# ChristophReich1996/Semantic_Pyramid_for_Image_Generation

Hardware: AMD Instinct MI355X
Metric: images/sec full G+D train step, 256x256, bs/GPU=20 (higher is better)
Workload: dtype bf16

## Files before the change

include/sempyr.h:

```cpp
#ifndef SEMPYR_H
#define SEMPYR_H
#include <stdint.h>

#ifdef __cplusplus
extern "C" {
#endif

#define SP_VERSION 1

typedef void* sp_stream_t;

enum sp_status { SP_OK = 0, SP_ERR_INVALID = -1, SP_ERR_LAUNCH = -2, SP_ERR_UNSUPPORTED = -3 };
enum sp_dtype { SP_F32 = 0, SP_BF16 = 1, SP_F8 = 2 ,
                SP_F16 = 3 ,
                SP_F8_F16 = 4  };
enum sp_act { SP_ACT_NONE = 0, SP_ACT_LRELU = 1, SP_ACT_RELU = 2, SP_ACT_TANH = 3 };

int sp_version(void);

enum { SP_TUNE_CONV_TALL = 0, SP_TUNE_IGEMM_DMA = 1, SP_TUNE_WGRAD_ROWS = 2, SP_TUNE_DETERMINISTIC = 3,
       SP_TUNE_SPLITK_TARGET = 4, SP_TUNE_SPLITK_MINSTEPS = 5, SP_TUNE_CONV1X1_DIRECT = 6, SP_TUNE_CONV_SHORT = 7,
       SP_TUNE_WGRAD9_BLOCKS = 8, SP_TUNE_WGRAD_BLOCKS = 9, SP_TUNE_WGRAD_MINSTEPS = 10, SP_TUNE_WGRAD_SMALL_M = 11,
       SP_TUNE_WGRAD_K1_TILE64 = 12, SP_TUNE_WGRAD_ROWS_THIN = 13, SP_TUNE_WGRAD_ROWS_BLOCKS = 14, SP_TUNE_WGRAD_ROWS_SLABS = 15,
       SP_TUNE_CONV_STAGGER = 16, SP_TUNE_CONV1X1_SPLITK = 17, SP_TUNE_WGRAD1X1 = 18, SP_TUNE_CONV_CIN8 = 19, SP_TUNE_CONV_THINCO = 20, SP_TUNE_CONV_PP = 21, SP_TUNE_CONV_PP_PRIO = 22, SP_TUNE_WGRAD_PP = 23, SP_TUNE_BN_ITERS = 24, SP_TUNE_IGEMM_TILE = 25, SP_TUNE_CONV_PPW = 26, SP_TUNE_LINEAR_KS = 27, SP_TUNE_CONV_PP_SPLIT = 28, SP_TUNE_PAIRSET_SEGMENTS = 29, SP_TUNE_ATTN_PIECES = 30, SP_TUNE_COUNT = 31 };
int sp_set_tuning(int32_t key, int32_t value);
const char* sp_last_error_string(void);
const char* sp_last_route(void);

typedef struct sp_conv_params {
    const void* x;
    const void* w;
    const float* bias;
    void* y;
    const void* res1;
    const void* res2;
    const void* mask_src;
    float mask_neg_slope;
    int32_t n, h, w_, cin_p, cout, ldy, ksize, act, dtype;
    void* workspace;
    int64_t workspace_bytes;
    int32_t pool2;
    int32_t in_up2;
    const float* x_scale;
    const float* w_scale;
    void* y8;
    const float* y8_inv_scale;
    float* y8_amax;
    const float* img_scale;
    int32_t img_split;
    int32_t reserved_;
    int64_t split_pix_;
    const void* tail_w;
    const float* tail_bias;
    void* tail_y;
    int32_t tail_cout, tail_act, tail_ld, reserved2_;
    uint32_t* pool_idx;
    int32_t* split_sync;
} sp_conv_params;
#define SP_CONV_SPLIT_SYNC_BYTES 8192
int sp_conv2d_igemm(const sp_conv_params* p, sp_stream_t stream);
int sp_conv2d_workspace(int32_t n, int32_t h, int32_t w_, int32_t cin_p, int32_t cout, int32_t ksize, int32_t dtype,
                        int64_t* bytes_out);
int sp_conv2d_route(const sp_conv_params* p, const char** route);

int sp_conv2d_wgrad(const void* x, const void* dy, float* dw, int32_t n, int32_t h, int32_t w_,
                    int32_t cin_p, int32_t cout, int32_t ld_dy, int32_t ksize, int32_t dtype,
                    sp_stream_t stream);

int sp_conv2d_wgrad_fused(const void* x, const void* dy, float* dw, float* dbias, const void* w_packed, float* dot,
                          float* workspace, int64_t workspace_floats, int32_t n, int32_t h, int32_t w_, int32_t cin_p,
                          int32_t cout, int32_t ld_dy, int32_t ksize, int32_t dtype, sp_stream_t stream);
int sp_conv2d_wgrad_accum(const void* x, const void* dy, float* dw, float* dbias, float* workspace, int64_t workspace_floats,
                          int32_t n, int32_t h, int32_t w_, int32_t cin_p, int32_t cout, int32_t ld_dy, int32_t ksize,
                          int32_t dtype, sp_stream_t stream);
int sp_conv2d_wgrad_accum_pooled(const void* x, const void* dy, float* dw, float* dbias, float* workspace, int64_t workspace_floats,
                                 int32_t n, int32_t h, int32_t w_, int32_t cin_p, int32_t cout, int32_t ld_dy, int32_t ksize,
                                 int32_t dtype, sp_stream_t stream);
int sp_conv2d_wgrad_workspace(int32_t n, int32_t h, int32_t w_, int32_t cin_p, int32_t cout, int32_t ksize,
                              int32_t dtype, int64_t* floats_out);
int sp_conv2d_wgrad_accum_pair(const void* x, const void* dy, float* dw_a, float* dbias_a, float* dw_b, float* dbias_b, float* workspace,
                               int64_t workspace_floats, int32_t n, int32_t split, int32_t h, int32_t w_, int32_t cin_p, int32_t cout,
                               int32_t ld_dy, int32_t ksize, int32_t dy_pooled, int32_t dtype, sp_stream_t stream);
int sp_conv2d_wgrad_route(int32_t n, int32_t split, int32_t h, int32_t w_, int32_t cin_p, int32_t cout, int32_t ld_dy, int32_t ksize,
                          int32_t dy_pooled, int32_t want_dbias, int64_t workspace_floats, int32_t dtype, const char** route);
int sp_wgrad_reduce_defer(int32_t on);
int sp_wgrad_reduce_flush(int32_t run, sp_stream_t stream);
int sp_wgrad_reduce_pending(void);

int sp_linear_fwd(const void* x, int32_t ldx, const void* w_packed, int32_t kp, const float* bias,
                  const void* res, void* y, int32_t ldy, int32_t batch, int32_t k, int32_t n, int32_t act,
                  int32_t dtype, sp_stream_t stream);
int sp_linear_workspace(int32_t batch, int32_t k, int32_t n, int32_t dtype, int64_t* floats_out);
int sp_linear_fwd_ws(const void* x, int32_t ldx, const void* w_packed, int32_t kp, const float* bias,
                     const void* res, void* y, int32_t ldy, int32_t batch, int32_t k, int32_t n, int32_t act,
                     int32_t dtype, float* scratch, sp_stream_t stream);
int sp_linear_wgrad(const void* x, int32_t ldx, const void* dy, int32_t ld_dy, float* dw, int32_t kp,
                    float* dbias, int32_t batch, int32_t k, int32_t n, int32_t dtype, sp_stream_t stream);

typedef struct sp_sn_layer {
    const float* w;
    float* u;
    float* v;
    int64_t scratch_off;
    int64_t part_off;
    int64_t fwd_off;
    int64_t dgrad_off;
    int32_t rows, cols, cin, taps, cin_p, cout_p, kind, pack_block0;
// ... 284 lines not shown
```

semantic_pyramid_for_image_generation_amd/_lib.py:

```python
from __future__ import annotations

import ctypes
import os
import re
from typing import Dict, List, Tuple

_HERE = os.path.dirname(os.path.abspath(__file__))
HEADER = os.path.join(os.path.dirname(_HERE), "include", "sempyr.h")
LIB_PATH = os.environ.get("SEMPYR_LIB") or os.path.join(_HERE, "libsempyr.so")

SP_F32, SP_BF16, SP_F8, SP_F16, SP_F8_F16 = 0, 1, 2, 3, 4
ACT_NONE, ACT_LRELU, ACT_RELU, ACT_TANH = 0, 1, 2, 3

TUNE_KEYS = {"SP_CONV_TALL": 0, "SP_IGEMM_DMA": 1, "SP_WGRAD_ROWS": 2, "SP_DETERMINISTIC": 3, "SP_SPLITK_TARGET": 4,
             "SP_SPLITK_MINSTEPS": 5, "SP_CONV1X1_DIRECT": 6, "SP_CONV_SHORT": 7, "SP_WGRAD9_BLOCKS": 8, "SP_WGRAD_BLOCKS": 9,
             "SP_WGRAD_MINSTEPS": 10, "SP_WGRAD_SMALL_M": 11, "SP_WGRAD_K1_TILE64": 12, "SP_WGRAD_ROWS_THIN": 13,
             "SP_WGRAD_ROWS_BLOCKS": 14, "SP_WGRAD_ROWS_SLABS": 15, "SP_CONV_STAGGER": 16, "SP_CONV1X1_SPLITK": 17, "SP_WGRAD1X1": 18, "SP_CONV_CIN8": 19, "SP_CONV_THINCO": 20,
             "SP_CONV_PP": 21, "SP_CONV_PP_PRIO": 22, "SP_WGRAD_PP": 23, "SP_BN_ITERS": 24, "SP_IGEMM_TILE": 25, "SP_CONV_PPW": 26, "SP_LINEAR_KS": 27, "SP_CONV_PP_SPLIT": 28, "SP_PAIRSET_SEGMENTS": 29, "SP_ATTN_PIECES": 30}


SP_CONV_SPLIT_SYNC_BYTES = 8192


class SpConvParams(ctypes.Structure):
    _fields_ = [("x", ctypes.c_void_p), ("w", ctypes.c_void_p), ("bias", ctypes.c_void_p), ("y", ctypes.c_void_p),
                ("res1", ctypes.c_void_p), ("res2", ctypes.c_void_p), ("mask_src", ctypes.c_void_p),
                ("mask_neg_slope", ctypes.c_float),
                ("n", ctypes.c_int32), ("h", ctypes.c_int32), ("w_", ctypes.c_int32), ("cin_p", ctypes.c_int32),
                ("cout", ctypes.c_int32), ("ldy", ctypes.c_int32), ("ksize", ctypes.c_int32), ("act", ctypes.c_int32),
                ("dtype", ctypes.c_int32), ("workspace", ctypes.c_void_p), ("workspace_bytes", ctypes.c_int64),
                ("pool2", ctypes.c_int32), ("in_up2", ctypes.c_int32),
                ("x_scale", ctypes.c_void_p), ("w_scale", ctypes.c_void_p), ("y8", ctypes.c_void_p),
                ("y8_inv_scale", ctypes.c_void_p), ("y8_amax", ctypes.c_void_p),
                ("img_scale", ctypes.c_void_p), ("img_split", ctypes.c_int32), ("reserved_", ctypes.c_int32),
                ("split_pix_", ctypes.c_int64),
                ("tail_w", ctypes.c_void_p), ("tail_bias", ctypes.c_void_p), ("tail_y", ctypes.c_void_p),
                ("tail_cout", ctypes.c_int32), ("tail_act", ctypes.c_int32), ("tail_ld", ctypes.c_int32), ("reserved2_", ctypes.c_int32),
                ("pool_idx", ctypes.c_void_p), ("split_sync", ctypes.c_void_p)]


class SpConvGeneralParams(ctypes.Structure):
    _fields_ = [("struct_bytes", ctypes.c_int32), ("dtype", ctypes.c_int32),
                ("x", ctypes.c_void_p), ("w", ctypes.c_void_p), ("bias", ctypes.c_void_p), ("y", ctypes.c_void_p),
                ("n", ctypes.c_int32), ("h", ctypes.c_int32), ("w_", ctypes.c_int32), ("cin_p", ctypes.c_int32),
                ("ldx", ctypes.c_int32), ("cout", ctypes.c_int32), ("ldy", ctypes.c_int32), ("kh", ctypes.c_int32),
                ("kw", ctypes.c_int32), ("stride_h", ctypes.c_int32), ("stride_w", ctypes.c_int32), ("pad_h", ctypes.c_int32),
                ("pad_w", ctypes.c_int32), ("act", ctypes.c_int32)]

    def __init__(self, **kw):
        super().__init__(struct_bytes=ctypes.sizeof(SpConvGeneralParams), **kw)


class SpSnLayer(ctypes.Structure):
    _fields_ = [("w", ctypes.c_void_p), ("u", ctypes.c_void_p), ("v", ctypes.c_void_p),
                ("scratch_off", ctypes.c_int64), ("part_off", ctypes.c_int64), ("fwd_off", ctypes.c_int64),
                ("dgrad_off", ctypes.c_int64),
                ("rows", ctypes.c_int32), ("cols", ctypes.c_int32), ("cin", ctypes.c_int32), ("taps", ctypes.c_int32),
                ("cin_p", ctypes.c_int32), ("cout_p", ctypes.c_int32), ("kind", ctypes.c_int32),
                ("pack_block0", ctypes.c_int32)]


class SpSnBwdLayer(ctypes.Structure):
    _fields_ = [("w", ctypes.c_void_p), ("dw_off", ctypes.c_int64), ("dot_off", ctypes.c_int64),
                ("scratch_off", ctypes.c_int64), ("grad_off", ctypes.c_int64),
                ("rows", ctypes.c_int32), ("cols", ctypes.c_int32), ("cin", ctypes.c_int32), ("taps", ctypes.c_int32),
                ("cin_p", ctypes.c_int32), ("plain", ctypes.c_int32), ("db_off", ctypes.c_int32),
                ("bias_off", ctypes.c_int32)]


class SpRecLevel(ctypes.Structure):
    _fields_ = [("real", ctypes.c_void_p), ("fake", ctypes.c_void_p), ("mask", ctypes.c_void_p), ("dfake", ctypes.c_void_p),
                ("ld_real", ctypes.c_int32), ("ld_fake", ctypes.c_int32), ("ld_dfake", ctypes.c_int32), ("n", ctypes.c_int32),
                ("h", ctypes.c_int32), ("w_", ctypes.c_int32), ("c", ctypes.c_int32), ("reserved_", ctypes.c_int32)]


_CTYPE = {"int32_t": ctypes.c_int32, "int64_t": ctypes.c_int64, "float": ctypes.c_float, "double": ctypes.c_double, "int": ctypes.c_int,
          "sp_stream_t": ctypes.c_void_p, "uint64_t": ctypes.c_uint64}


def parse_header(path: str = HEADER) -> Dict[str, Tuple[object, List[object]]]:
    text = open(path).read()
    text = re.sub(r"/\*.*?\*/", "", text, flags=re.S)
    protos = {}
    for m in re.finditer(r"\b(int|const char\*)\s+(sp_\w+)\s*\(([^;{]*?)\)\s*;", text, flags=re.S):
        ret, name, args = m.group(1), m.group(2), m.group(3).strip()
        argtypes = []
        if args and args != "void":
            for a in args.split(","):
                a = " ".join(a.split())
                if "*" in a:
                    argtypes.append(ctypes.c_void_p)
                else:
                    ty = a.rsplit(" ", 1)[0].replace("const ", "").strip()
                    argtypes.append(_CTYPE[ty])
        protos[name] = (ctypes.c_char_p if "char" in ret else ctypes.c_int, argtypes)
    return protos


class SempyrError(RuntimeError):
    pass

# ... 48 lines not shown
```

semantic_pyramid_for_image_generation_amd/csrc/conv_igemm.hip:

```cpp
#include "conv_common.h"

namespace {

template <typename T, int WCO, int WPX, int FCO, int FPX>
__global__ __launch_bounds__(256) void conv_igemm_kernel(sp_conv_params p) {
    constexpr int CO_T = WCO * FCO * 16, PX_T = WPX * FPX * 16;
    constexpr int E = 16 / (int)sizeof(T);
    constexpr int KC = 8 * E;
    constexpr int W_CH = CO_T * 8, X_CH = PX_T * 8;
    constexpr int W_PER = (W_CH + 255) / 256, X_PER = (X_CH + 255) / 256;
    constexpr int STAGE = (CO_T + PX_T) * 128;
    extern __shared__ __attribute__((aligned(16))) char smem[];

    const int tid = threadIdx.x, lane = tid & 63, wave = tid >> 6;
    const int wco = wave / WPX, wpx = wave % WPX;
    const int H = p.h, W = p.w_, CIN = p.cin_p;
    const long M = (long)p.n * H * W;
    const long px0 = (long)blockIdx.x * PX_T;
    const int co0 = blockIdx.y * CO_T;
    const int taps = p.ksize * p.ksize;
    const int kchunks = (CIN + KC - 1) / KC;
    const int nk = taps * kchunks;
    const T* __restrict__ xg = reinterpret_cast<const T*>(p.x);
    const T* __restrict__ wg = reinterpret_cast<const T*>(p.w);
// ... 1073 lines not shown
    const bf16* __restrict__ xg = reinterpret_cast<const bf16*>(p.x);
    const bf16* __restrict__ wg = reinterpret_cast<const bf16*>(p.w);
    const int ksteps = (CIN + 31) / 32;
    const int per = (ksteps + 3) / 4;
    const int m0 = wave * per;
    const int cnt = ksteps - m0 < per ? ksteps - m0 : per;
    const int i16 = lane & 15, g = lane >> 4;
    const int arow = (i16 >> 2) * 16 + (i16 & 3);
    const long px0 = (long)blockIdx.x * 32 + i16, px1 = px0 + 16;
    const bf16* x0 = xg + (px0 < M ? px0 : M - 1) * CIN + g * 8;
    const bf16* x1 = xg + (px1 < M ? px1 : M - 1) * CIN + g * 8;
    const bf16* wr[4];
#pragma unroll
    for (int i = 0; i < 4; ++i) {
        const int row = co0 + arow + i * 4;
        wr[i] = wg + (long)(row < p.cout ? row : p.cout - 1) * CIN + g * 8;
    }
    f32x4_t acc[4][2];
#pragma unroll
    for (int i = 0; i < 4; ++i) { acc[i][0] = f32x4_t{0.f, 0.f, 0.f, 0.f}; acc[i][1] = f32x4_t{0.f, 0.f, 0.f, 0.f}; }
    for (int c0 = 0; c0 < cnt; c0 += KMAX) {
        uint4 a[KMAX][4], b[KMAX][2];
        static_for<KMAX>([&](auto uc) {
            constexpr int u = decltype(uc)::value;
            const int m = m0 + c0 + u;
#pragma unroll
            for (int i = 0; i < 4; ++i) a[u][i] = make_uint4(0, 0, 0, 0);
            b[u][0] = make_uint4(0, 0, 0, 0);
            b[u][1] = make_uint4(0, 0, 0, 0);
            if (c0 + u < cnt && m * 32 + g * 8 < CIN) {
#pragma unroll
                for (int i = 0; i < 4; ++i) a[u][i] = *reinterpret_cast<const uint4*>(wr[i] + m * 32);
                b[u][0] = *reinterpret_cast<const uint4*>(x0 + m * 32);
                b[u][1] = *reinterpret_cast<const uint4*>(x1 + m * 32);
            }
        });
        static_for<KMAX>([&](auto uc) {
            constexpr int u = decltype(uc)::value;
            if (c0 + u < cnt) {
#pragma unroll
                for (int i = 0; i < 4; ++i) {
                    acc[i][0] = __builtin_amdgcn_mfma_f32_16x16x32_bf16(__builtin_bit_cast(bf16x8_t, a[u][i]), __builtin_bit_cast(bf16x8_t, b[u][0]), acc[i][0], 0, 0, 0);
                    acc[i][1] = __builtin_amdgcn_mfma_f32_16x16x32_bf16(__builtin_bit_cast(bf16x8_t, a[u][i]), __builtin_bit_cast(bf16x8_t, b[u][1]), acc[i][1], 0, 0, 0);
                }
            }
        });
    }
#pragma unroll
    for (int i = 0; i < 4; ++i)
#pragma unroll
        for (int j = 0; j < 2; ++j)
            red[((wave * 4 + i) * 2 + j) * 64 + lane] = make_float4(acc[i][j][0], acc[i][j][1], acc[i][j][2], acc[i][j][3]);
    __syncthreads();
    const bool vec_ok = ((p.ldy & 3) == 0) && ((p.cout & 3) == 0);
    const int co = co0 + g * 16 + wave * 4;
    if (co >= p.cout) return;
#pragma unroll
    for (int j = 0; j < 2; ++j) {
        const long pix = j == 0 ? px0 : px1;
        float v[4] = {0.f, 0.f, 0.f, 0.f};
#pragma unroll
        for (int src = 0; src < 4; ++src) {
            const float4 t = red[((src * 4 + wave) * 2 + j) * 64 + lane];
            v[0] += t.x; v[1] += t.y; v[2] += t.z; v[3] += t.w;
        }
        if (pix < M) conv_epilogue4<bf16>(p, v, pix, co, vec_ok);
    }
}

int launch_1x1_splitk(const sp_conv_params& p, hipStream_t s) {
    const int ksteps = (p.cin_p + 31) / 32;
    const long M = (long)p.n * p.h * p.w_;
    dim3 grid((unsigned)((M + 31) / 32), (unsigned)((p.cout + 63) / 64));
    sp_note_route(conv_route_name(CK_1X1_SPLITK, 0, false));
    if (ksteps <= 8) hipLaunchKernelGGL(conv1x1_splitk_kernel<2>, grid, dim3(256), 0, s, p);
    else if (ksteps <= 16) hipLaunchKernelGGL(conv1x1_splitk_kernel<4>, grid, dim3(256), 0, s, p);
    else hipLaunchKernelGGL(conv1x1_splitk_kernel<6>, grid, dim3(256), 0, s, p);
    SP_LAUNCH_CHECK();
    return SP_OK;
}

constexpr int C8_TH = 16, C8_TW = 32, C8_HW = C8_TW + 2, C8_HH = C8_TH + 2;

__global__ __launch_bounds__(256) void conv3x3_cin8_kernel(sp_conv_params p) {
    __shared__ __attribute__((aligned(16))) uint4 halo[C8_HH * C8_HW];
    const int tid = threadIdx.x, lane = tid & 63, wave = tid >> 6;
    const int H = p.h, W = p.w_;
    const int tiles_x = W / C8_TW, tiles_y = H / C8_TH;
    int t = blockIdx.x;
    const int tx0 = (t % tiles_x) * C8_TW; t /= tiles_x;
    const int ty0 = (t % tiles_y) * C8_TH;
    const int n = t / tiles_y;
    const uint4* __restrict__ xg = reinterpret_cast<const uint4*>(p.x);
    const uint4* __restrict__ wg = reinterpret_cast<const uint4*>(p.w);
    uint4 hv[3];
#pragma unroll
    for (int q = 0; q < 3; ++q) {
        const int e = tid + q * 256;
        const int r = e / C8_HW, c = e - r * C8_HW;
        const int y = ty0 - 1 + r, x = tx0 - 1 + c;
        hv[q] = make_uint4(0, 0, 0, 0);
        if (e < C8_HH * C8_HW && (unsigned)y < (unsigned)H && (unsigned)x < (unsigned)W) hv[q] = xg[((long)n * H + y) * W + x];
    }
    const int i16 = lane & 15, g = lane >> 4;
    uint4 a[4][3];
#pragma unroll
    for (int i = 0; i < 4; ++i) {
        const int co = (i16 >> 2) * 16 + i * 4 + (i16 & 3);
#pragma unroll
        for (int m = 0; m < 3; ++m) {
            const int tap = m * 4 + g;
            a[i][m] = make_uint4(0, 0, 0, 0);
            if (tap < 9 && co < p.cout) a[i][m] = wg[co * 9 + tap];
        }
    }
#pragma unroll
    for (int q = 0; q < 3; ++q) {
        const int e = tid + q * 256;
        if (e < C8_HH * C8_HW) halo[e] = hv[q];
    }
    __syncthreads();
    int toff[3];
#pragma unroll
    for (int m = 0; m < 3; ++m) {
        const int tap = m * 4 + g < 9 ? m * 4 + g : 8;
        toff[m] = (tap / 3) * C8_HW + tap % 3;
    }
    const int co_b = g * 16;
    const bool co_ok = co_b + 16 <= p.cout;
    float bias[16];
#pragma unroll
    for (int r = 0; r < 16; ++r) bias[r] = 0.f;
    if (p.bias && co_ok) Wide16<float>::ld(p.bias + co_b, bias);
#pragma unroll 2
    for (int rr = 0; rr < C8_TH / 4; ++rr) {
        const int row = wave * (C8_TH / 4) + rr;
        f32x4_t acc[4][2];
#pragma unroll
        for (int i = 0; i < 4; ++i) { acc[i][0] = f32x4_t{0.f, 0.f, 0.f, 0.f}; acc[i][1] = f32x4_t{0.f, 0.f, 0.f, 0.f}; }
#pragma unroll
        for (int m = 0; m < 3; ++m) {
            const uint4 b0 = halo[row * C8_HW + i16 + toff[m]];
            const uint4 b1 = halo[row * C8_HW + 16 + i16 + toff[m]];
#pragma unroll
            for (int i = 0; i < 4; ++i) {
                acc[i][0] = __builtin_amdgcn_mfma_f32_16x16x32_bf16(__builtin_bit_cast(bf16x8_t, a[i][m]), __builtin_bit_cast(bf16x8_t, b0), acc[i][0], 0, 0, 0);
                acc[i][1] = __builtin_amdgcn_mfma_f32_16x16x32_bf16(__builtin_bit_cast(bf16x8_t, a[i][m]), __builtin_bit_cast(bf16x8_t, b1), acc[i][1], 0, 0, 0);
            }
        }
        if (!co_ok) continue;
        const long pix0 = ((long)n * H + ty0 + row) * W + tx0 + i16;
        const float sc = conv_img_scale(p, pix0);
#pragma unroll
        for (int j = 0; j < 2; ++j) {
            float v[16];
#pragma unroll
            for (int i = 0; i < 4; ++i)
#pragma unroll
                for (int r = 0; r < 4; ++r) v[i * 4 + r] = acc[i][j][r] * sc + bias[i * 4 + r];
            conv_epilogue16<bf16>(p, v, pix0 + j * 16, co_b, false);
        }
    }
}

int launch_cin8(const sp_conv_params& p, hipStream_t s) {
    const long blocks = (long)p.n * (p.h / C8_TH) * (p.w_ / C8_TW);
    sp_note_route(conv_route_name(CK_CIN8, 0, false));
    hipLaunchKernelGGL(conv3x3_cin8_kernel, dim3((unsigned)blocks), dim3(256), 0, s, p);
    SP_LAUNCH_CHECK();
    return SP_OK;
}

constexpr int TN_TH = 8, TN_TW = 32, TN_HW = TN_TW + 2, TN_HH = TN_TH + 2;

template <int KC>
__global__ __launch_bounds__(256) void conv3x3_thinco_kernel(sp_conv_params p) {
    extern __shared__ __attribute__((aligned(16))) char tn_smem[];
    constexpr int CIN = KC * 32, PITCH = CIN * 2 + 16, CPP = KC * 4;
    constexpr int NCH = TN_HH * TN_HW * CPP, PER = (NCH + 255) / 256;
    const int tid = threadIdx.x, lane = tid & 63, wave = tid >> 6;
    const int H = p.h, W = p.w_;
    const int tiles_x = W / TN_TW, tiles_y = H / TN_TH;
    int t = blockIdx.x;
    const int tx0 = (t % tiles_x) * TN_TW; t /= tiles_x;
    const int ty0 = (t % tiles_y) * TN_TH;
    const int n = t / tiles_y;
    const uint4* __restrict__ xg = reinterpret_cast<const uint4*>(p.x);
    const uint4* __restrict__ wg = reinterpret_cast<const uint4*>(p.w);
    uint4 hv[PER];
#pragma unroll
    for (int q = 0; q < PER; ++q) {
        const int e = tid + q * 256;
        const int px = e / CPP, c = e - px * CPP;
        const int r = px / TN_HW, cc = px - r * TN_HW;
        const int y = ty0 - 1 + r, x = tx0 - 1 + cc;
        hv[q] = make_uint4(0, 0, 0, 0);
        if (e < NCH && (unsigned)y < (unsigned)H && (unsigned)x < (unsigned)W) hv[q] = xg[(((long)n * H + y) * W + x) * CPP + c];
    }
    const int i16 = lane & 15, g = lane >> 4;
    uint4 a[9][KC];
#pragma unroll
    for (int tap = 0; tap < 9; ++tap)
#pragma unroll
        for (int kc = 0; kc < KC; ++kc) {
            a[tap][kc] = make_uint4(0, 0, 0, 0);
            if (i16 < p.cout) a[tap][kc] = wg[(i16 * 9 + tap) * CPP + kc * 4 + g];
        }
#pragma unroll
    for (int q = 0; q < PER; ++q) {
        const int e = tid + q * 256;
        const int px = e / CPP, c = e - px * CPP;
        if (e < NCH) *reinterpret_cast<uint4*>(tn_smem + px * PITCH + c * 16) = hv[q];
    }
    __syncthreads();
    const bool vec_ok = ((p.ldy & 3) == 0) && ((p.cout & 3) == 0);
#pragma unroll
    for (int rr = 0; rr < TN_TH / 4; ++rr) {
        const int row = wave * (TN_TH / 4) + rr;
        f32x4_t acc[2] = {f32x4_t{0.f, 0.f, 0.f, 0.f}, f32x4_t{0.f, 0.f, 0.f, 0.f}};
#pragma unroll
        for (int tap = 0; tap < 9; ++tap) {
            const char* base = tn_smem + ((row + tap / 3) * TN_HW + i16 + tap % 3) * PITCH + g * 16;
#pragma unroll
            for (int kc = 0; kc < KC; ++kc) {
                const uint4 b0 = *reinterpret_cast<const uint4*>(base + kc * 64);
                const uint4 b1 = *reinterpret_cast<const uint4*>(base + 16 * PITCH + kc * 64);
                acc[0] = __builtin_amdgcn_mfma_f32_16x16x32_bf16(__builtin_bit_cast(bf16x8_t, a[tap][kc]), __builtin_bit_cast(bf16x8_t, b0), acc[0], 0, 0, 0);
                acc[1] = __builtin_amdgcn_mfma_f32_16x16x32_bf16(__builtin_bit_cast(bf16x8_t, a[tap][kc]), __builtin_bit_cast(bf16x8_t, b1), acc[1], 0, 0, 0);
            }
        }
        if (g != 0) continue;
        const long pix0 = ((long)n * H + ty0 + row) * W + tx0 + i16;
#pragma unroll
        for (int j = 0; j < 2; ++j) {
            float v[4] = {acc[j][0], acc[j][1], acc[j][2], acc[j][3]};
            conv_epilogue4<bf16>(p, v, pix0 + j * 16, 0, vec_ok);
        }
    }
}

template <int KC>
int launch_thinco(const sp_conv_params& p, hipStream_t s) {
    constexpr int LDS = TN_HH * TN_HW * (KC * 64 + 16);
    if (const int rc = sp_lds_limit<conv3x3_thinco_kernel<KC>>(LDS)) return rc;
    const long blocks = (long)p.n * (p.h / TN_TH) * (p.w_ / TN_TW);
    sp_note_route(conv_route_name(CK_THINCO, 0, false));
    hipLaunchKernelGGL(conv3x3_thinco_kernel<KC>, dim3((unsigned)blocks), dim3(256), LDS, s, p);
    SP_LAUNCH_CHECK();
    return SP_OK;
}

// ... 200 lines not shown
```

semantic_pyramid_for_image_generation_amd/csrc/eltwise.hip:

```cpp
#include "common.h"

namespace {

inline int grid_for(long work_items) {
    long b = (work_items + 255) / 256;
    if (b > 2048) b = 2048;
    if (b < 1) b = 1;
    return (int)b;
}

__device__ __forceinline__ float fl32(float v) {
    asm("" : "+v"(v));
    return v;
}

template <typename TS, typename TD>
__global__ void ingest_kernel(const TS* __restrict__ src, long sn, long sc, long sh, long sw, TD* __restrict__ dst,
                              int N, int C, int H, int W, int CP, float3 scale, float3 shift) {
    const long total = (long)N * H * W;
    for (long p = (long)blockIdx.x * 256 + threadIdx.x; p < total; p += (long)gridDim.x * 256) {
        const int w = (int)(p % W);
        const long q = p / W;
        const int h = (int)(q % H);
        const int n = (int)(q / H);
        const TS* s = src + n * sn + h * sh + w * sw;
        const float sc3[3] = {scale.x, scale.y, scale.z}, sf3[3] = {shift.x, shift.y, shift.z};
        for (int c = 0; c < CP; ++c) {
            float v = 0.f;
            if (c < C) v = Elem<TS>::ld(s + c * sc) * sc3[c % 3] + sf3[c % 3];
            Elem<TD>::st(dst + p * CP + c, fl32(v));
        }
    }
}

template <typename T>
__global__ void ingest_bwd_kernel(const T* __restrict__ dy, int CP, T* __restrict__ dsrc, int C, long pixels, float3 scale) {
    const float sc3[3] = {scale.x, scale.y, scale.z};
    for (long p = (long)blockIdx.x * 256 + threadIdx.x; p < pixels; p += (long)gridDim.x * 256)
        for (int c = 0; c < C; ++c) Elem<T>::st(dsrc + p * C + c, fl32(Elem<T>::ld(dy + p * CP + c) * sc3[c % 3]));
}

template <typename T>
__global__ void mask_concat_kernel(const T* __restrict__ feat, const float* __restrict__ mask, T* __restrict__ out,
                                   long pixels, int C, int CP) {
    const int vpp = CP / 4;
    const long total = pixels * vpp;
    for (long i = (long)blockIdx.x * 256 + threadIdx.x; i < total; i += (long)gridDim.x * 256) {
        const long p = i / vpp;
        const int c = (int)(i - p * vpp) * 4;
        const float m = mask[p];
        float v[4] = {0.f, 0.f, 0.f, 0.f};
        if (c + 3 < C) {
            Elem<T>::ld4(feat + p * C + c, v);
#pragma unroll
            for (int r = 0; r < 4; ++r) v[r] *= m;
        } else {
#pragma unroll
            for (int r = 0; r < 4; ++r) {
                if (c + r < C) v[r] = Elem<T>::ld(feat + p * C + c + r) * m;
                else if (c + r == C) v[r] = m;
            }
        }
        Elem<T>::st4(out + p * CP + c, v);
    }
}

template <typename T>
__global__ void mask_mul_2d_kernel(const T* __restrict__ feat, int ldf, const float* __restrict__ mask, T* __restrict__ out,
                                   int ldo, int B, int K) {
    const long total = (long)B * ldo;
    for (long i = (long)blockIdx.x * 256 + threadIdx.x; i < total; i += (long)gridDim.x * 256) {
        const int b = (int)(i / ldo), k = (int)(i % ldo);
        float v = 0.f;
        if (k < K) v = Elem<T>::ld(feat + (long)b * ldf + k) * mask[(long)b * K + k];
        Elem<T>::st(out + i, fl32(v));
    }
}

template <typename T>
__global__ void act_fwd_kernel(const T* __restrict__ x, T* __restrict__ y, long n4, int act) {
    for (long i = (long)blockIdx.x * 256 + threadIdx.x; i < n4; i += (long)gridDim.x * 256) {
        float v[4];
        Elem<T>::ld4(x + i * 4, v);
        apply_act_vec<4>(v, act);
        Elem<T>::st4(y + i * 4, v);
    }
}

__device__ __forceinline__ float act_grad(float dy, float y, int act) {
    if (act == SP_ACT_LRELU) return y > 0.f ? dy : 0.2f * dy;
    if (act == SP_ACT_RELU) return y > 0.f ? dy : 0.f;
    if (act == SP_ACT_TANH) return dy * (1.f - y * y);
    return dy;
}

template <typename T>
__global__ void act_bwd_kernel(const T* __restrict__ dy, const T* __restrict__ y, T* __restrict__ dz, long n4, int act) {
    for (long i = (long)blockIdx.x * 256 + threadIdx.x; i < n4; i += (long)gridDim.x * 256) {
        float d[4], v[4];
        Elem<T>::ld4(dy + i * 4, d);
        Elem<T>::ld4(y + i * 4, v);
#pragma unroll
        for (int r = 0; r < 4; ++r) d[r] = act_grad(d[r], v[r], act);
        Elem<T>::st4(dz + i * 4, d);
    }
}

template <typename T>
__global__ void act_bwd_pad_kernel(const T* __restrict__ dy, const T* __restrict__ y, T* __restrict__ dz, long pixels,
                                   int C, int CP, int act) {
    const long total = pixels * CP;
    for (long i = (long)blockIdx.x * 256 + threadIdx.x; i < total; i += (long)gridDim.x * 256) {
        const long p = i / CP;
// ... 62 lines not shown
    }
    const float tot = block_sum_256(part, red);
    if (threadIdx.x == 0) dg_part[blockIdx.x] = tot;
}

__global__ __launch_bounds__(256) void column_sum_kernel(const float* __restrict__ part, int rows, int cols, float* __restrict__ out) {
    __shared__ float red[4];
    const int col = blockIdx.x;
    float t = 0.f;
    for (int r = threadIdx.x; r < rows; r += 256) t += part[(long)r * cols + col];
    const float tot = block_sum_256(t, red);
    if (threadIdx.x == 0) out[col] = tot;
}

template <typename T>
__global__ void permute_kernel(const T* __restrict__ src, T* __restrict__ dst, int B, int C, int HW, int to_hwc) {
    const long total = (long)B * C * HW;
    for (long i = (long)blockIdx.x * 256 + threadIdx.x; i < total; i += (long)gridDim.x * 256) {
        const int b = (int)(i / ((long)C * HW));
        const int r = (int)(i - (long)b * C * HW);
        long s;
        if (to_hwc) { const int hw = r / C, c = r - hw * C; s = (long)b * C * HW + (long)c * HW + hw; }
        else { const int c = r / HW, hw = r - c * HW; s = (long)b * C * HW + (long)hw * C + c; }
        dst[i] = src[s];
    }
}

template <typename T>
__global__ __launch_bounds__(256) void channel_sum_kernel(const T* __restrict__ x, int ld, long pixels, int C,
                                                          float* __restrict__ out) {
    __shared__ float red[256 * 4];
    const int ngroups = (C + 3) / 4;
    const int lanes_per_pix = ngroups < 256 ? ngroups : 256;
    const int pix_par = 256 / lanes_per_pix;
    const int cg = threadIdx.x % lanes_per_pix, pl = threadIdx.x / lanes_per_pix;
    const bool vec = (ld & 3) == 0;
    for (int cbase = 0; cbase < ngroups; cbase += lanes_per_pix) {
        const int c = (cbase + cg) * 4;
        float acc[4] = {0.f, 0.f, 0.f, 0.f};
        const bool live = c < C && pl < pix_par;
        if (live) {
            for (long p = (long)blockIdx.x * pix_par + pl; p < pixels; p += (long)gridDim.x * pix_par) {
                if (vec) {
                    float v[4];
                    Elem<T>::ld4(x + p * ld + c, v);
                    acc[0] += v[0]; acc[1] += v[1]; acc[2] += v[2]; acc[3] += v[3];
                } else {
                    for (int r = 0; r < 4 && c + r < C; ++r) acc[r] += Elem<T>::ld(x + p * ld + c + r);
                }
            }
        }
        __syncthreads();
#pragma unroll
        for (int r = 0; r < 4; ++r) red[threadIdx.x * 4 + r] = acc[r];
        __syncthreads();
        if (live && pl == 0) {
            for (int r = 0; r < 4 && c + r < C; ++r) {
                float t = 0.f;
                for (int k = 0; k < pix_par; ++k) t += red[(k * lanes_per_pix + cg) * 4 + r];
                out[(long)blockIdx.x * C + c + r] = t;
            }
        }
    }
}

}

#define SP_CHECK_DTYPE(dtype, name) do { if ((dtype) != SP_F32 && (dtype) != SP_BF16) { \
    sp_set_error("%s: dtype %d not supported (SP_F32 / SP_BF16 / SP_F16)", name, (int)(dtype)); return SP_ERR_UNSUPPORTED; } } while (0)
#define SP_CHECK_ACT(act, name) do { if ((act) < SP_ACT_NONE || (act) > SP_ACT_TANH) { \
    sp_set_error("%s: act %d not supported (SP_ACT_NONE / LRELU / RELU / TANH)", name, (int)(act)); return SP_ERR_UNSUPPORTED; } } while (0)
#define SP_DT_SWITCH(dtype, CALL_F32, CALL_BF16) do { if ((dtype) == SP_F32) { CALL_F32; } else { CALL_BF16; } } while (0)

extern "C" int sp_ingest_image(const void* src, int32_t src_dtype, int64_t sn, int64_t sc, int64_t sh, int64_t sw,
                               void* dst, int32_t n, int32_t c, int32_t h, int32_t w_, int32_t cp, const float* scale3,
                               const float* shift3, int32_t dtype, sp_stream_t stream) {
    SP_CHECK_ARG(src && dst && c <= 3 && cp >= c, "sp_ingest_image: bad args");
    SP_CHECK_ARG(src_dtype == SP_F32 || src_dtype == SP_BF16, "sp_ingest_image: bad src_dtype %d", (int)src_dtype);
    SP_CHECK_DTYPE(dtype, "sp_ingest_image");
    hipStream_t s = reinterpret_cast<hipStream_t>(stream);
    float3 sc3 = make_float3(1.f, 1.f, 1.f), sf3 = make_float3(0.f, 0.f, 0.f);
    if (scale3) sc3 = make_float3(scale3[0], scale3[1], scale3[2]);
    if (shift3) sf3 = make_float3(shift3[0], shift3[1], shift3[2]);
    const int g = grid_for((long)n * h * w_);
    if (src_dtype == SP_F32 && dtype == SP_F32)
        hipLaunchKernelGGL((ingest_kernel<float, float>), dim3(g), dim3(256), 0, s, (const float*)src, sn, sc, sh, sw, (float*)dst, n, c, h, w_, cp, sc3, sf3);
    else if (src_dtype == SP_F32 && dtype == SP_BF16)
        hipLaunchKernelGGL((ingest_kernel<float, bf16>), dim3(g), dim3(256), 0, s, (const float*)src, sn, sc, sh, sw, (bf16*)dst, n, c, h, w_, cp, sc3, sf3);
    else if (src_dtype == SP_BF16 && dtype == SP_BF16)
        hipLaunchKernelGGL((ingest_kernel<bf16, bf16>), dim3(g), dim3(256), 0, s, (const bf16*)src, sn, sc, sh, sw, (bf16*)dst, n, c, h, w_, cp, sc3, sf3);
    else
        hipLaunchKernelGGL((ingest_kernel<bf16, float>), dim3(g), dim3(256), 0, s, (const bf16*)src, sn, sc, sh, sw, (float*)dst, n, c, h, w_, cp, sc3, sf3);
    SP_LAUNCH_CHECK();
    return SP_OK;
}

extern "C" int sp_ingest_image_bwd(const void* dy, int32_t cp, void* dsrc, int32_t c, int64_t pixels, const float* scale3,
                                   int32_t dtype, sp_stream_t stream) {
    SP_CHECK_ARG(dy && dsrc && c <= 3 && cp >= c, "sp_ingest_image_bwd: bad args");
    SP_CHECK_DTYPE(dtype, "sp_ingest_image_bwd");
    hipStream_t s = reinterpret_cast<hipStream_t>(stream);
    float3 sc3 = make_float3(1.f, 1.f, 1.f);
    if (scale3) sc3 = make_float3(scale3[0], scale3[1], scale3[2]);
    const int g = grid_for(pixels);
    SP_DT_SWITCH(dtype,
                 hipLaunchKernelGGL(ingest_bwd_kernel<float>, dim3(g), dim3(256), 0, s, (const float*)dy, cp, (float*)dsrc, c, (long)pixels, sc3),
                 hipLaunchKernelGGL(ingest_bwd_kernel<bf16>, dim3(g), dim3(256), 0, s, (const bf16*)dy, cp, (bf16*)dsrc, c, (long)pixels, sc3));
    SP_LAUNCH_CHECK();
    return SP_OK;
}

extern "C" int sp_mask_concat(const void* feat, const float* mask, void* out, int64_t pixels, int32_t c, int32_t cp,
                              int32_t dtype, sp_stream_t stream) {
    SP_CHECK_ARG(feat && mask && out && cp > c && cp % 4 == 0 && c % 4 == 0, "sp_mask_concat: bad args (c=%d cp=%d)", c, cp);
    SP_CHECK_DTYPE(dtype, "sp_mask_concat");
    hipStream_t s = reinterpret_cast<hipStream_t>(stream);
    const int g = grid_for(pixels * (cp / 4));
    SP_DT_SWITCH(dtype,
                 hipLaunchKernelGGL(mask_concat_kernel<float>, dim3(g), dim3(256), 0, s, (const float*)feat, mask, (float*)out, (long)pixels, c, cp),
                 hipLaunchKernelGGL(mask_concat_kernel<bf16>, dim3(g), dim3(256), 0, s, (const bf16*)feat, mask, (bf16*)out, (long)pixels, c, cp));
    SP_LAUNCH_CHECK();
    return SP_OK;
}

extern "C" int sp_mask_mul_2d(const void* feat, int32_t ldf, const float* mask, void* out, int32_t ldo, int32_t batch,
                              int32_t k, int32_t dtype, sp_stream_t stream) {
    SP_CHECK_ARG(feat && mask && out && ldf >= k && ldo >= k, "sp_mask_mul_2d: bad args");
    SP_CHECK_DTYPE(dtype, "sp_mask_mul_2d");
    hipStream_t s = reinterpret_cast<hipStream_t>(stream);
    const int g = grid_for((long)batch * ldo);
    SP_DT_SWITCH(dtype,
                 hipLaunchKernelGGL(mask_mul_2d_kernel<float>, dim3(g), dim3(256), 0, s, (const float*)feat, ldf, mask, (float*)out, ldo, batch, k),
                 hipLaunchKernelGGL(mask_mul_2d_kernel<bf16>, dim3(g), dim3(256), 0, s, (const bf16*)feat, ldf, mask, (bf16*)out, ldo, batch, k));
    SP_LAUNCH_CHECK();
    return SP_OK;
}

extern "C" int sp_act_fwd(const void* x, void* y, int64_t numel, int32_t act, int32_t dtype, sp_stream_t stream) {
    SP_CHECK_ARG(x && y && numel % 4 == 0, "sp_act_fwd: numel must be a multiple of 4");
    SP_CHECK_DTYPE(dtype, "sp_act_fwd");
    SP_CHECK_ACT(act, "sp_act_fwd");
    hipStream_t s = reinterpret_cast<hipStream_t>(stream);
    const int g = grid_for(numel / 4);
    SP_DT_SWITCH(dtype,
                 hipLaunchKernelGGL(act_fwd_kernel<float>, dim3(g), dim3(256), 0, s, (const float*)x, (float*)y, (long)(numel / 4), act),
                 hipLaunchKernelGGL(act_fwd_kernel<bf16>, dim3(g), dim3(256), 0, s, (const bf16*)x, (bf16*)y, (long)(numel / 4), act));
    SP_LAUNCH_CHECK();
    return SP_OK;
}

extern "C" int sp_act_bwd(const void* dy, const void* y, void* dz, int64_t pixels, int32_t c, int32_t cp, int32_t act,
                          int32_t dtype, sp_stream_t stream) {
    SP_CHECK_ARG(dy && y && dz && cp >= c, "sp_act_bwd: bad args");
    SP_CHECK_DTYPE(dtype, "sp_act_bwd");
    SP_CHECK_ACT(act, "sp_act_bwd");
    hipStream_t s = reinterpret_cast<hipStream_t>(stream);
    if (c == cp && (pixels * c) % 4 == 0) {
        const long n4 = pixels * c / 4;
        const int g = grid_for(n4);
        SP_DT_SWITCH(dtype,
                     hipLaunchKernelGGL(act_bwd_kernel<float>, dim3(g), dim3(256), 0, s, (const float*)dy, (const float*)y, (float*)dz, n4, act),
                     hipLaunchKernelGGL(act_bwd_kernel<bf16>, dim3(g), dim3(256), 0, s, (const bf16*)dy, (const bf16*)y, (bf16*)dz, n4, act));
    } else {
        const int g = grid_for(pixels * cp);
        SP_DT_SWITCH(dtype,
                     hipLaunchKernelGGL(act_bwd_pad_kernel<float>, dim3(g), dim3(256), 0, s, (const float*)dy, (const float*)y, (float*)dz, (long)pixels, c, cp, act),
// ... 188 lines not shown
```

Measured before the change: 1408.

## Make cin8 3x3 conv persistent with double-buffered halo; row-wise image ingest

The 8-channel 3x3 conv kernel becomes persistent: a capped grid (tunable, default 3 blocks per CU) walks contiguous tiles. It prefetches the next tile's halo into registers and stages it into a second LDS buffer while computing the current one, and keeps the weights and bias loaded once per block. Separately, image ingest into 8-channel padded layout gets a row-oriented kernel with coalesced column access, 16-byte stores and several rows in flight per thread. The goal is to cut per-tile launch and weight-reload overhead and to overlap global loads with MFMA work, at the cost of doubled LDS, an occupancy hint and extra control logic.

Result: no change. 1416, median of 6 (+0.5%).

```diff
diff --git a/include/sempyr.h b/include/sempyr.h
--- a/include/sempyr.h
+++ b/include/sempyr.h
@@ -22,7 +22,7 @@
        SP_TUNE_SPLITK_TARGET = 4, SP_TUNE_SPLITK_MINSTEPS = 5, SP_TUNE_CONV1X1_DIRECT = 6, SP_TUNE_CONV_SHORT = 7,
        SP_TUNE_WGRAD9_BLOCKS = 8, SP_TUNE_WGRAD_BLOCKS = 9, SP_TUNE_WGRAD_MINSTEPS = 10, SP_TUNE_WGRAD_SMALL_M = 11,
        SP_TUNE_WGRAD_K1_TILE64 = 12, SP_TUNE_WGRAD_ROWS_THIN = 13, SP_TUNE_WGRAD_ROWS_BLOCKS = 14, SP_TUNE_WGRAD_ROWS_SLABS = 15,
-       SP_TUNE_CONV_STAGGER = 16, SP_TUNE_CONV1X1_SPLITK = 17, SP_TUNE_WGRAD1X1 = 18, SP_TUNE_CONV_CIN8 = 19, SP_TUNE_CONV_THINCO = 20, SP_TUNE_CONV_PP = 21, SP_TUNE_CONV_PP_PRIO = 22, SP_TUNE_WGRAD_PP = 23, SP_TUNE_BN_ITERS = 24, SP_TUNE_IGEMM_TILE = 25, SP_TUNE_CONV_PPW = 26, SP_TUNE_LINEAR_KS = 27, SP_TUNE_CONV_PP_SPLIT = 28, SP_TUNE_PAIRSET_SEGMENTS = 29, SP_TUNE_ATTN_PIECES = 30, SP_TUNE_COUNT = 31 };
+       SP_TUNE_CONV_STAGGER = 16, SP_TUNE_CONV1X1_SPLITK = 17, SP_TUNE_WGRAD1X1 = 18, SP_TUNE_CONV_CIN8 = 19, SP_TUNE_CONV_THINCO = 20, SP_TUNE_CONV_PP = 21, SP_TUNE_CONV_PP_PRIO = 22, SP_TUNE_WGRAD_PP = 23, SP_TUNE_BN_ITERS = 24, SP_TUNE_IGEMM_TILE = 25, SP_TUNE_CONV_PPW = 26, SP_TUNE_LINEAR_KS = 27, SP_TUNE_CONV_PP_SPLIT = 28, SP_TUNE_PAIRSET_SEGMENTS = 29, SP_TUNE_ATTN_PIECES = 30, SP_TUNE_CIN8_GRID = 31, SP_TUNE_COUNT = 32 };
 int sp_set_tuning(int32_t key, int32_t value);
 const char* sp_last_error_string(void);
 const char* sp_last_route(void);
diff --git a/semantic_pyramid_for_image_generation_amd/_lib.py b/semantic_pyramid_for_image_generation_amd/_lib.py
--- a/semantic_pyramid_for_image_generation_amd/_lib.py
+++ b/semantic_pyramid_for_image_generation_amd/_lib.py
@@ -16,7 +16,8 @@
              "SP_SPLITK_MINSTEPS": 5, "SP_CONV1X1_DIRECT": 6, "SP_CONV_SHORT": 7, "SP_WGRAD9_BLOCKS": 8, "SP_WGRAD_BLOCKS": 9,
              "SP_WGRAD_MINSTEPS": 10, "SP_WGRAD_SMALL_M": 11, "SP_WGRAD_K1_TILE64": 12, "SP_WGRAD_ROWS_THIN": 13,
              "SP_WGRAD_ROWS_BLOCKS": 14, "SP_WGRAD_ROWS_SLABS": 15, "SP_CONV_STAGGER": 16, "SP_CONV1X1_SPLITK": 17, "SP_WGRAD1X1": 18, "SP_CONV_CIN8": 19, "SP_CONV_THINCO": 20,
-             "SP_CONV_PP": 21, "SP_CONV_PP_PRIO": 22, "SP_WGRAD_PP": 23, "SP_BN_ITERS": 24, "SP_IGEMM_TILE": 25, "SP_CONV_PPW": 26, "SP_LINEAR_KS": 27, "SP_CONV_PP_SPLIT": 28, "SP_PAIRSET_SEGMENTS": 29, "SP_ATTN_PIECES": 30}
+             "SP_CONV_PP": 21, "SP_CONV_PP_PRIO": 22, "SP_WGRAD_PP": 23, "SP_BN_ITERS": 24, "SP_IGEMM_TILE": 25, "SP_CONV_PPW": 26, "SP_LINEAR_KS": 27, "SP_CONV_PP_SPLIT": 28, "SP_PAIRSET_SEGMENTS": 29, "SP_ATTN_PIECES": 30,
+             "SP_CIN8_GRID": 31}
 
 
 SP_CONV_SPLIT_SYNC_BYTES = 8192
diff --git a/semantic_pyramid_for_image_generation_amd/csrc/conv_igemm.hip b/semantic_pyramid_for_image_generation_amd/csrc/conv_igemm.hip
--- a/semantic_pyramid_for_image_generation_amd/csrc/conv_igemm.hip
+++ b/semantic_pyramid_for_image_generation_amd/csrc/conv_igemm.hip
@@ -1179,26 +1179,47 @@
 
 constexpr int C8_TH = 16, C8_TW = 32, C8_HW = C8_TW + 2, C8_HH = C8_TH + 2;
 
-__global__ __launch_bounds__(256) void conv3x3_cin8_kernel(sp_conv_params p) {
-    __shared__ __attribute__((aligned(16))) uint4 halo[C8_HH * C8_HW];
+__global__ __launch_bounds__(256, 3) void conv3x3_cin8_kernel(sp_conv_params p, int tiles) {
+    __shared__ __attribute__((aligned(16))) uint4 c8_smem[2 * C8_HH * C8_HW + 16];
+    uint4 (*halo)[C8_HH * C8_HW] = reinterpret_cast<uint4 (*)[C8_HH * C8_HW]>(c8_smem);
+    float* sbias = reinterpret_cast<float*>(c8_smem + 2 * C8_HH * C8_HW);
     const int tid = threadIdx.x, lane = tid & 63, wave = tid >> 6;
+    if (tid < 64) sbias[tid] = (p.bias && tid < p.cout) ? p.bias[tid] : 0.f;
     const int H = p.h, W = p.w_;
     const int tiles_x = W / C8_TW, tiles_y = H / C8_TH;
-    int t = blockIdx.x;
-    const int tx0 = (t % tiles_x) * C8_TW; t /= tiles_x;
-    const int ty0 = (t % tiles_y) * C8_TH;
-    const int n = t / tiles_y;
+    const int per = tiles / (int)gridDim.x, rem = tiles % (int)gridDim.x;
+    const int b = blockIdx.x;
+    const int count = per + (b < rem ? 1 : 0);
+    int t = b * per + (b < rem ? b : rem);
+    int tx0 = (t % tiles_x) * C8_TW; t /= tiles_x;
+    int ty0 = (t % tiles_y) * C8_TH;
+    int n = t / tiles_y;
     const uint4* __restrict__ xg = reinterpret_cast<const uint4*>(p.x);
     const uint4* __restrict__ wg = reinterpret_cast<const uint4*>(p.w);
-    uint4 hv[3];
+    int hr[3], hc[3];
 #pragma unroll
     for (int q = 0; q < 3; ++q) {
         const int e = tid + q * 256;
-        const int r = e / C8_HW, c = e - r * C8_HW;
-        const int y = ty0 - 1 + r, x = tx0 - 1 + c;
-        hv[q] = make_uint4(0, 0, 0, 0);
-        if (e < C8_HH * C8_HW && (unsigned)y < (unsigned)H && (unsigned)x < (unsigned)W) hv[q] = xg[((long)n * H + y) * W + x];
-    }
+        hr[q] = e / C8_HW - 1;
+        hc[q] = e - (e / C8_HW) * C8_HW - 1;
+    }
+    const auto fetch = [&](uint4 (&hv)[3], int fn, int fy0, int fx0) {
+#pragma unroll
+        for (int q = 0; q < 3; ++q) {
+            const int y = fy0 + hr[q], x = fx0 + hc[q];
+            hv[q] = make_uint4(0, 0, 0, 0);
+            if (tid + q * 256 < C8_HH * C8_HW && (unsigned)y < (unsigned)H && (unsigned)x < (unsigned)W) hv[q] = xg[((long)fn * H + y) * W + x];
+        }
+    };
+    const auto stage = [&](const uint4 (&hv)[3], int buf) {
+#pragma unroll
+        for (int q = 0; q < 3; ++q) {
+            const int e = tid + q * 256;
+            if (e < C8_HH * C8_HW) halo[buf][e] = hv[q];
+        }
+    };
+    uint4 hv[3];
+    fetch(hv, n, ty0, tx0);
     const int i16 = lane & 15, g = lane >> 4;
     uint4 a[4][3];
 #pragma unroll
@@ -1211,11 +1232,7 @@
             if (tap < 9 && co < p.cout) a[i][m] = wg[co * 9 + tap];
         }
     }
-#pragma unroll
-    for (int q = 0; q < 3; ++q) {
-        const int e = tid + q * 256;
-        if (e < C8_HH * C8_HW) halo[e] = hv[q];
-    }
+    stage(hv, 0);
     __syncthreads();
     int toff[3];
 #pragma unroll
@@ -1225,45 +1242,57 @@
     }
     const int co_b = g * 16;
     const bool co_ok = co_b + 16 <= p.cout;
-    float bias[16];
-#pragma unroll
-    for (int r = 0; r < 16; ++r) bias[r] = 0.f;
-    if (p.bias && co_ok) Wide16<float>::ld(p.bias + co_b, bias);
-#pragma unroll 2
-    for (int rr = 0; rr < C8_TH / 4; ++rr) {
-        const int row = wave * (C8_TH / 4) + rr;
-        f32x4_t acc[4][2];
-#pragma unroll
-        for (int i = 0; i < 4; ++i) { acc[i][0] = f32x4_t{0.f, 0.f, 0.f, 0.f}; acc[i][1] = f32x4_t{0.f, 0.f, 0.f, 0.f}; }
-#pragma unroll
-        for (int m = 0; m < 3; ++m) {
-            const uint4 b0 = halo[row * C8_HW + i16 + toff[m]];
-            const uint4 b1 = halo[row * C8_HW + 16 + i16 + toff[m]];
-#pragma unroll
-            for (int i = 0; i < 4; ++i) {
-                acc[i][0] = __builtin_amdgcn_mfma_f32_16x16x32_bf16(__builtin_bit_cast(bf16x8_t, a[i][m]), __builtin_bit_cast(bf16x8_t, b0), acc[i][0], 0, 0, 0);
-                acc[i][1] = __builtin_amdgcn_mfma_f32_16x16x32_bf16(__builtin_bit_cast(bf16x8_t, a[i][m]), __builtin_bit_cast(bf16x8_t, b1), acc[i][1], 0, 0, 0);
-            }
-        }
-        if (!co_ok) continue;
-        const long pix0 = ((long)n * H + ty0 + row) * W + tx0 + i16;
-        const float sc = conv_img_scale(p, pix0);
-#pragma unroll
-        for (int j = 0; j < 2; ++j) {
-            float v[16];
-#pragma unroll
-            for (int i = 0; i < 4; ++i)
-#pragma unroll
-                for (int r = 0; r < 4; ++r) v[i * 4 + r] = acc[i][j][r] * sc + bias[i * 4 + r];
-            conv_epilogue16<bf16>(p, v, pix0 + j * 16, co_b, false);
-        }
+    for (int it = 0; it < count; ++it) {
+        const int cur = it & 1;
+        int nx0 = tx0 + C8_TW, ny0 = ty0, nn = n;
+        if (nx0 == W) {
+            nx0 = 0;
+            ny0 += C8_TH;
+            if (ny0 == H) { ny0 = 0; ++nn; }
+        }
+        const bool more = it + 1 < count;
+        if (more) fetch(hv, nn, ny0, nx0);
+        for (int rr = 0; rr < C8_TH / 4; ++rr) {
+            const int row = wave * (C8_TH / 4) + rr;
+            const long pix0 = ((long)n * H + ty0 + row) * W + tx0 + i16;
+            const float sc = conv_img_scale(p, pix0);
+            static_for<2>([&](auto jc) {
+                constexpr int j = decltype(jc)::value;
+                f32x4_t acc[4];
+#pragma unroll
+                for (int i = 0; i < 4; ++i) acc[i] = f32x4_t{0.f, 0.f, 0.f, 0.f};
+#pragma unroll
+                for (int m = 0; m < 3; ++m) {
+                    const uint4 bj = halo[cur][row * C8_HW + j * 16 + i16 + toff[m]];
+#pragma unroll
+                    for (int i = 0; i < 4; ++i)
+                        acc[i] = __builtin_amdgcn_mfma_f32_16x16x32_bf16(__builtin_bit_cast(bf16x8_t, a[i][m]), __builtin_bit_cast(bf16x8_t, bj), acc[i], 0, 0, 0);
+                }
+                if (co_ok) {
+                    float bias[16], v[16];
+                    Wide16<float>::ld(sbias + co_b, bias);
+#pragma unroll
+                    for (int i = 0; i < 4; ++i)
+#pragma unroll
+                        for (int r = 0; r < 4; ++r) v[i * 4 + r] = acc[i][r] * sc + bias[i * 4 + r];
+                    conv_epilogue16<bf16>(p, v, pix0 + j * 16, co_b, false);
+                }
+            });
+        }
+        if (!more) break;
+        stage(hv, cur ^ 1);
+        __syncthreads();
+        tx0 = nx0; ty0 = ny0; n = nn;
     }
 }
 
 int launch_cin8(const sp_conv_params& p, hipStream_t s) {
-    const long blocks = (long)p.n * (p.h / C8_TH) * (p.w_ / C8_TW);
+    const long tiles = (long)p.n * (p.h / C8_TH) * (p.w_ / C8_TW);
+    if (tiles > 0x7fffffffL) { sp_set_error("sp_conv2d_igemm: too many 16x32 tiles for the 8-channel 3x3 kernel"); return SP_ERR_UNSUPPORTED; }
+    const int cap = sp_tune(SP_TUNE_CIN8_GRID, 3 * NUM_CU);
+    const long blocks = tiles < cap ? tiles : (cap < 1 ? 1 : cap);
     sp_note_route(conv_route_name(CK_CIN8, 0, false));
-    hipLaunchKernelGGL(conv3x3_cin8_kernel, dim3((unsigned)blocks), dim3(256), 0, s, p);
+    hipLaunchKernelGGL(conv3x3_cin8_kernel, dim3((unsigned)blocks), dim3(256), 0, s, p, (int)tiles);
     SP_LAUNCH_CHECK();
     return SP_OK;
 }
diff --git a/semantic_pyramid_for_image_generation_amd/csrc/eltwise.hip b/semantic_pyramid_for_image_generation_amd/csrc/eltwise.hip
--- a/semantic_pyramid_for_image_generation_amd/csrc/eltwise.hip
+++ b/semantic_pyramid_for_image_generation_amd/csrc/eltwise.hip
@@ -29,6 +29,51 @@
             float v = 0.f;
             if (c < C) v = Elem<TS>::ld(s + c * sc) * sc3[c % 3] + sf3[c % 3];
             Elem<TD>::st(dst + p * CP + c, fl32(v));
+        }
+    }
+}
+
+__device__ __forceinline__ void ingest_st8(bf16* d, float v0, float v1, float v2) {
+    *reinterpret_cast<uint4*>(d) = make_uint4(f32x2_to_bf16x2(v0, v1), f32x2_to_bf16x2(v2, 0.f), 0u, 0u);
+}
+__device__ __forceinline__ void ingest_st8(float* d, float v0, float v1, float v2) {
+    *reinterpret_cast<float4*>(d) = make_float4(v0, v1, v2, 0.f);
+    *reinterpret_cast<float4*>(d + 4) = make_float4(0.f, 0.f, 0.f, 0.f);
+}
+
+constexpr int INGEST_ROWS_DEPTH = 4;
+template <typename TS, typename TD>
+__global__ __launch_bounds__(256) void ingest_rows_kernel(const TS* __restrict__ src, long sn, long sc, long sh, long sw,
+                                                          TD* __restrict__ dst, int C, int H, int W, long rows, int LW,
+                                                          int step_n, int step_h, float3 scale, float3 shift) {
+    constexpr int D = INGEST_ROWS_DEPTH;
+    const int cols = 1 << LW, col = threadIdx.x & (cols - 1);
+    long row = (long)blockIdx.x * (256 >> LW) + (threadIdx.x >> LW);
+    if (row >= rows) return;
+    const long step = (long)step_n * H + step_h;
+    int n = (int)(row / H), h = (int)(row - (long)n * H);
+    const float sc3[3] = {scale.x, scale.y, scale.z}, sf3[3] = {shift.x, shift.y, shift.z};
+    for (; row < rows; row += D * step) {
+        const TS* s[D];
+#pragma unroll
+        for (int k = 0; k < D; ++k) {
+            s[k] = src + n * sn + h * sh;
+            n += step_n;
+            h += step_h;
+            if (h >= H) { h -= H; ++n; }
+        }
+        for (int w = col; w < W; w += cols) {
+            float v[D][3];
+#pragma unroll
+            for (int k = 0; k < D; ++k)
+#pragma unroll
+                for (int c = 0; c < 3; ++c) {
+                    v[k][c] = 0.f;
+                    if (c < C && row + k * step < rows) v[k][c] = Elem<TS>::ld(s[k] + w * sw + c * sc) * sc3[c] + sf3[c];
+                }
+#pragma unroll
+            for (int k = 0; k < D; ++k)
+                if (row + k * step < rows) ingest_st8(dst + ((row + k * step) * W + w) * 8, fl32(v[k][0]), fl32(v[k][1]), fl32(v[k][2]));
         }
     }
 }
@@ -257,6 +302,25 @@
     float3 sc3 = make_float3(1.f, 1.f, 1.f), sf3 = make_float3(0.f, 0.f, 0.f);
     if (scale3) sc3 = make_float3(scale3[0], scale3[1], scale3[2]);
     if (shift3) sf3 = make_float3(shift3[0], shift3[1], shift3[2]);
+    const long rows = (long)n * h;
+    if (cp == 8 && rows > 0 && w_ > 0 && reinterpret_cast<uintptr_t>(dst) % 16 == 0) {
+        int lw = 0;
+        while (lw < 8 && (1 << lw) < w_) ++lw;
+        const int rpb = 256 >> lw;
+        long g = ((rows + rpb - 1) / rpb + INGEST_ROWS_DEPTH - 1) / INGEST_ROWS_DEPTH;
+        if (g > 2048) g = 2048;
+        const long step = g * rpb;
+        const int step_n = (int)(step / h), step_h = (int)(step % h);
+#define SP_INGEST_ROWS(TS, TD) hipLaunchKernelGGL((ingest_rows_kernel<TS, TD>), dim3((unsigned)g), dim3(256), 0, s, (const TS*)src, sn, sc, sh, sw, \
+                                                  (TD*)dst, c, h, w_, rows, lw, step_n, step_h, sc3, sf3)
+        if (src_dtype == SP_F32 && dtype == SP_F32) SP_INGEST_ROWS(float, float);
+        else if (src_dtype == SP_F32 && dtype == SP_BF16) SP_INGEST_ROWS(float, bf16);
+        else if (src_dtype == SP_BF16 && dtype == SP_BF16) SP_INGEST_ROWS(bf16, bf16);
+        else SP_INGEST_ROWS(bf16, float);
+#undef SP_INGEST_ROWS
+        SP_LAUNCH_CHECK();
+        return SP_OK;
+    }
     const int g = grid_for((long)n * h * w_);
     if (src_dtype == SP_F32 && dtype == SP_F32)
         hipLaunchKernelGGL((ingest_kernel<float, float>), dim3(g), dim3(256), 0, s, (const float*)src, sn, sc, sh, sw, (float*)dst, n, c, h, w_, cp, sc3, sf3);
```
